# bowang-lab/BioReason

Hardware: AMD Instinct MI355X
Metric: GRPO samples/sec (NT-500M+Qwen3-1.7B, DNA 2x1024, prompt 2180, gen 256) (higher is better)
Workload: dtype bf16

## Files before the change

### bioreason_amd/csrc/bra_decattn.h

```cpp
#pragma once
#include "bra_device.h"
#include "bra_gridsync.h"

namespace bra {


constexpr float kNegA = -1.0e30f;
constexpr float kLog2eA = 1.4426950408889634f;

struct DecOneArgs {
    const bf16_t* qkv; long ldqkv;
    const bf16_t* qw; const bf16_t* kw;
    const float* cosT; const float* sinT;
    const int* pos;
    const float* rope_rows;
    const bf16_t* kp; long kp_sr, kp_sh, kp_ss;
    const bf16_t* vtp; long vt_sr, vt_sh, vt_sd;
    const uint8_t* pmask;
    bf16_t* kc;
    bf16_t* vct; long cp;
    float* part_o; float* part_ml;
    bf16_t* o; long ldo;
    int R, copies, Hq, Hkv, P, C, t, nslot, npc, ncc_grid;
    float eps, scale;
    const int* t_ptr;
    float inv_Hq, inv_npc, inv_Hkv, inv_ncc, inv_copies;
    int rsplit; float inv_rsplit;
};

__device__ __forceinline__ int da_div(int w, float inv) { return (int)(((float)w + 0.5f) * inv); }
#ifdef BRA_EMU
__device__ __forceinline__ unsigned da_mul24(int a, int b) { return ((unsigned)a & 0xffffffu) * ((unsigned)b & 0xffffffu); }
#else
__device__ __forceinline__ unsigned da_mul24(int a, int b) { return __umul24((unsigned)a, (unsigned)b); }
#endif

template <int HD>
__device__ __forceinline__ void nr_slice(float (&x)[8], const bf16_t* nw, const float* cosr, const float* sinr, int dl, float eps) {
    constexpr int LPK = HD / 8;
    float ss = 0.f;
#pragma unroll
    for (int i = 0; i < 8; ++i) ss += x[i] * x[i];
#pragma unroll
    for (int mk = LPK >> 1; mk >= 1; mk >>= 1) ss += wave_shfl_xor(ss, mk);
    const float rstd = rsqrtf(ss / (float)HD + eps);
    float w[8];
    unpack8(ld16(nw + dl * 8), w);
#pragma unroll
    for (int i = 0; i < 8; ++i) x[i] = round_bf(w[i] * round_bf(x[i] * rstd));
    const int hsl = (dl & (LPK / 2 - 1)) * 8;
    const bool upper = dl >= LPK / 2;
    const f32x4 c0 = *reinterpret_cast<const f32x4*>(cosr + hsl), c1 = *reinterpret_cast<const f32x4*>(cosr + hsl + 4);
    const f32x4 s0 = *reinterpret_cast<const f32x4*>(sinr + hsl), s1 = *reinterpret_cast<const f32x4*>(sinr + hsl + 4);
#pragma unroll
    for (int i = 0; i < 8; ++i) {
        const float other = wave_shfl_xor(x[i], LPK / 2);
        const float c = i < 4 ? c0[i & 3] : c1[i & 3], s = i < 4 ? s0[i & 3] : s1[i & 3];
        x[i] = round_bf(upper ? x[i] * c + other * s : x[i] * c - other * s);
    }
}

template <int HD>
__device__ __forceinline__ void item_kv_issue(const bf16_t* kbase, const int kss, const bf16_t* vbase, const int vsd, const int key0,
                                              const int nkeys, u32x4 (&kf)[4][HD / 32], u32x4 (&vf)[HD / 16][2]) {
    constexpr int DS = HD / 32, DB = HD / 16;
    const int lane = lane_id();
    const int fr = lane & 15, fq = lane >> 4;
#pragma unroll
    for (int kb = 0; kb < 4; ++kb) {
        int key = key0 + 32 * (kb >> 1) + 8 * (fr >> 2) + 4 * (kb & 1) + (fr & 3);
        key = key < nkeys ? key : nkeys - 1;
        const bf16_t* kr = kbase + (da_mul24(key, kss) + (unsigned)(fq * 8));
#pragma unroll
        for (int s = 0; s < DS; ++s) kf[kb][s] = ld16(kr + s * 32);
    }
    const unsigned vlane = da_mul24(fr, vsd) + (unsigned)(key0 + fq * 8);
#pragma unroll
    for (int db = 0; db < DB; ++db) {
        const bf16_t* vr = vbase + (long)db * 16 * vsd + vlane;
#pragma unroll
        for (int kk = 0; kk < 2; ++kk) vf[db][kk] = ld16(vr + kk * 32);
    }
}

template <int HD, int G, int XS = 0, int PRE = 0>
__device__ __forceinline__ void one_item(const DecOneArgs& a, const bf16_t* kbase, const int kss, const bf16_t* vbase, const int vsd,
                                         const int key0, const int nkeys, const uint8_t* mask, const int r, const int hkv,
                                         const int row_lo, const int row_hi, const int slot,
                                         u32x4 (&kf)[4][HD / 32], u32x4 (&vf)[HD / 16][2]) {
    constexpr int DS = HD / 32;
    constexpr int DB = HD / 16;
    const int lane = lane_id();
    const int fr = lane & 15, fq = lane >> 4;
    const int rows = a.copies * G;
    const int qrow = fr < rows ? fr : rows - 1;
    const int copy = (int)((unsigned)qrow / (unsigned)G), g = (int)((unsigned)qrow % (unsigned)G);
    const int b = r * a.copies + copy, hq = hkv * G + g;
    const unsigned qoff = da_mul24(b, (int)a.ldqkv) + (unsigned)(hq * HD);
    u32x4 qraw[DS], qwv[DS];
#pragma unroll
    for (int s = 0; s < DS; ++s) qraw[s] = xld16<XS>(a.qkv, (qoff + (unsigned)(s * 32 + fq * 8)) * 2u);
#pragma unroll
    for (int s = 0; s < DS; ++s) qwv[s] = ld16(a.qw + s * 32 + fq * 8);
    const float* cosr; const float* sinr;
    if (a.rope_rows) { cosr = a.rope_rows + (unsigned)(b * HD); sinr = cosr + HD / 2; }
    else { const int p = a.pos[b]; cosr = a.cosT + (long)p * (HD / 2); sinr = a.sinT + (long)p * (HD / 2); }
    f32x4 cs[DS / 2][4];
#pragma unroll
    for (int s = 0; s < DS / 2; ++s) {
        const int hb = s * 32 + fq * 8;
        cs[s][0] = *reinterpret_cast<const f32x4*>(cosr + hb); cs[s][1] = *reinterpret_cast<const f32x4*>(cosr + hb + 4);
        cs[s][2] = *reinterpret_cast<const f32x4*>(sinr + hb); cs[s][3] = *reinterpret_cast<const f32x4*>(sinr + hb + 4);
    }
    const bool nomask = mask == nullptr;
    uint8_t mb;
    {
        const int key = key0 + lane;
        const uint8_t* mp = nomask ? reinterpret_cast<const uint8_t*>(a.qw) : mask + (unsigned)(key < nkeys ? key : nkeys - 1);
        mb = *mp;
    }
    if constexpr (PRE == 0) item_kv_issue<HD>(kbase, kss, vbase, vsd, key0, nkeys, kf, vf);
    uint64_t vbits;
    {
        const int key = key0 + lane;
        vbits = wave_ballot((key < nkeys) & (nomask | (mb != 0)));
    }
    sched_fence();
    float qv[DS][8];
    float ss = 0.f;
#pragma unroll
    for (int s = 0; s < DS; ++s) {
        unpack8(qraw[s], qv[s]);
#pragma unroll
        for (int i = 0; i < 8; ++i) ss += qv[s][i] * qv[s][i];
    }
    ss += wave_shfl_xor(ss, 16);
    ss += wave_shfl_xor(ss, 32);
    const float rstd = rsqrtf(ss / (float)HD + a.eps);
#pragma unroll
    for (int s = 0; s < DS; ++s) {
        float w[8];
        unpack8(qwv[s], w);
#pragma unroll
        for (int i = 0; i < 8; ++i) qv[s][i] = round_bf(w[i] * round_bf(qv[s][i] * rstd));
    }
    const float sc = a.scale * kLog2eA;
    u32x4 qf[DS];
#pragma unroll
    for (int s = 0; s < DS; ++s) {
        const bool upper = s >= DS / 2;
        const int sp = s ^ (DS / 2), sh = s & (DS / 2 - 1);
        float o[8];
#pragma unroll
        for (int i = 0; i < 8; ++i) {
            const float cv = i < 4 ? cs[sh][0][i & 3] : cs[sh][1][i & 3], sv = i < 4 ? cs[sh][2][i & 3] : cs[sh][3][i & 3];
            const float rot = upper ? qv[s][i] * cv + qv[sp][i] * sv : qv[s][i] * cv - qv[sp][i] * sv;
            o[i] = round_bf(rot) * sc;
        }
        qf[s] = pack8(o);
    }
    f32x4 sreg[4];
    float m = kNegA;
#pragma unroll
    for (int kb = 0; kb < 4; ++kb) {
        f32x4 acc = {0.f, 0.f, 0.f, 0.f};
#pragma unroll
        for (int s = 0; s < DS; ++s) acc = mfma_16x16x32(kf[kb][s], qf[s], acc);
#pragma unroll
        for (int j = 0; j < 4; ++j) {
            const int rel_ = 32 * (kb >> 1) + 8 * fq + 4 * (kb & 1) + j;
            const bool ok = (vbits >> rel_) & 1ull;
            acc[j] = ok ? acc[j] : kNegA;
            m = fmaxf(m, acc[j]);
        }
        sreg[kb] = acc;
    }
    m = fmaxf(m, wave_shfl_xor(m, 16));
    m = fmaxf(m, wave_shfl_xor(m, 32));
    float l = 0.f;
#pragma unroll
    for (int kb = 0; kb < 4; ++kb)
#pragma unroll
        for (int j = 0; j < 4; ++j) {
            const float pe = sreg[kb][j] > 0.5f * kNegA ? fast_exp2(sreg[kb][j] - m) : 0.f;
            sreg[kb][j] = pe;
            l += pe;
        }
    l += wave_shfl_xor(l, 16);
    l += wave_shfl_xor(l, 32);
    const unsigned base = da_mul24((int)da_mul24(b, a.Hq) + hq, a.nslot) + (unsigned)slot;
    const bool live = fr < rows && fr >= row_lo && fr < row_hi;
#pragma unroll
    for (int db = 0; db < DB; ++db) {
        f32x4 acc = {0.f, 0.f, 0.f, 0.f};
#pragma unroll
        for (int kk = 0; kk < 2; ++kk) {
            u32x4 pf;
            pf.x = pack_bf2(sreg[2 * kk][0], sreg[2 * kk][1]);
            pf.y = pack_bf2(sreg[2 * kk][2], sreg[2 * kk][3]);
            pf.z = pack_bf2(sreg[2 * kk + 1][0], sreg[2 * kk + 1][1]);
            pf.w = pack_bf2(sreg[2 * kk + 1][2], sreg[2 * kk + 1][3]);
            acc = mfma_16x16x32(vf[db][kk], pf, acc);
        }
        if (live) xst16<XS>(a.part_o, (base * HD + (unsigned)(db * 16 + 4 * fq)) * 4u, __builtin_bit_cast(u32x4, acc));
    }
    if (live && fq == 0) {
        u32x2 mlv; mlv.x = __builtin_bit_cast(uint32_t, m); mlv.y = __builtin_bit_cast(uint32_t, l);
        xst8<XS>(a.part_ml, base * 8u, mlv);
    }
}

template <int HD, int G, int XS = 0>
__device__ __forceinline__ void one_newkey(const DecOneArgs& a, const int b, const int hq, const int t) {
    constexpr int LPK = HD / 8;
    const int lane = lane_id();
    const int grp = lane / LPK, dl = lane % LPK;
    const int hkv = hq / G;
    const int Nq = a.Hq * HD, Nkv = a.Hkv * HD;
    const int which = grp == 1 ? 1 : (grp == 2 ? 2 : 0);
    const unsigned src = da_mul24(b, (int)a.ldqkv) + (unsigned)(which == 0 ? hq * HD : (which == 1 ? Nq + hkv * HD : Nq + Nkv + hkv * HD));
    float x[8], y[8];
    unpack8(xld16<XS>(a.qkv, (src + (unsigned)(dl * 8)) * 2u), x);
    const float* cosr; const float* sinr;
    if (a.rope_rows) { cosr = a.rope_rows + (long)b * HD; sinr = cosr + HD / 2; }
    else { const int p = a.pos[b]; cosr = a.cosT + (long)p * (HD / 2); sinr = a.sinT + (long)p * (HD / 2); }
#pragma unroll
    for (int i = 0; i < 8; ++i) y[i] = x[i];
    nr_slice<HD>(y, which == 1 ? a.kw : a.qw, cosr, sinr, dl, a.eps);
    float d = 0.f;
#pragma unroll
    for (int i = 0; i < 8; ++i) d += y[i] * wave_shfl_xor(y[i], LPK);
#pragma unroll
    for (int mk = LPK >> 1; mk >= 1; mk >>= 1) d += wave_shfl_xor(d, mk);
    const float s_new = wave_shfl(d, 0) * a.scale * kLog2eA;
    if (hq % G == 0) {
        if (grp == 1) st16(a.kc + (((long)b * a.Hkv + hkv) * a.C + t) * HD + dl * 8, pack8(y));
        if (grp == 2) {
            bf16_t* vp = a.vct + (((long)b * a.Hkv + hkv) * HD + dl * 8) * a.cp + t;
#pragma unroll
            for (int i = 0; i < 8; ++i) vp[(long)i * a.cp] = f2bf(x[i]);
        }
    }
    const unsigned base = (unsigned)((b * a.Hq + hq) * a.nslot + a.npc + (t + 63) / 64);
    if (grp == 2) {
        const unsigned ob = (base * HD + (unsigned)(dl * 8)) * 4u;
        xst16<XS>(a.part_o, ob, __builtin_bit_cast(u32x4, f32x4{x[0], x[1], x[2], x[3]}));
        xst16<XS>(a.part_o, ob + 16u, __builtin_bit_cast(u32x4, f32x4{x[4], x[5], x[6], x[7]}));
    }
    if (lane == 0) {
        u32x2 mlv; mlv.x = __builtin_bit_cast(uint32_t, s_new); mlv.y = __builtin_bit_cast(uint32_t, 1.f);
        xst8<XS>(a.part_ml, base * 8u, mlv);
    }
}

struct DecItem {
    int kind;
    int b, hq;
    const bf16_t* kbase; int kss; const bf16_t* vbase; int vsd; int key0, nkeys; const uint8_t* mask;
    int r, hkv, row_lo, row_hi, slot;
};

template <int HD, int G>
__device__ __forceinline__ void dec_item_decode(const DecOneArgs& a, int w, const int t, DecItem& d) {
    const int nK = a.R * a.copies * a.Hq;
    const int nP = a.npc * a.Hkv * a.R;
    d.kind = 0;
    if (w >= nK && w < nK + nP) {
        w -= nK;
        const int q1 = da_div(w, a.inv_npc), c = w - q1 * a.npc;
        const int r = da_div(q1, a.inv_Hkv), hkv = q1 - r * a.Hkv;
        const int rp = a.rsplit > 1 ? da_div(r, a.inv_rsplit) : r;
        d.kind = 2;
        d.kbase = a.kp + rp * a.kp_sr + hkv * a.kp_sh; d.kss = (int)a.kp_ss;
        d.vbase = a.vtp + rp * a.vt_sr + hkv * a.vt_sh; d.vsd = (int)a.vt_sd;
        d.key0 = c * 64; d.nkeys = a.P; d.mask = a.pmask ? a.pmask + (long)rp * a.P : nullptr;
        d.r = r; d.hkv = hkv; d.row_lo = 0; d.row_hi = 16; d.slot = c;
        return;
    }
    if (w < nK) {
        d.kind = 1;
        d.b = da_div(w, a.inv_Hq);
        d.hq = w - d.b * a.Hq;
        return;
    }
    {
        const int v = w - nK - nP;
        const int q1 = da_div(v, a.inv_ncc), c = v - q1 * a.ncc_grid;
        const int q2 = da_div(q1, a.inv_copies), copy = q1 - q2 * a.copies;
        const int r = da_div(q2, a.inv_Hkv), hkv = q2 - r * a.Hkv;
        if (c * 64 >= t || r >= a.R) return;
        const int b = r * a.copies + copy;
        d.kind = 2;
        d.kbase = a.kc + ((long)b * a.Hkv + hkv) * a.C * HD; d.kss = HD;
        d.vbase = a.vct + ((long)b * a.Hkv + hkv) * HD * a.cp; d.vsd = (int)a.cp;
        d.key0 = c * 64; d.nkeys = t; d.mask = nullptr;
        d.r = r; d.hkv = hkv; d.row_lo = copy * G; d.row_hi = copy * G + G; d.slot = a.npc + c;
    }
}

template <int HD, int G, int XS, int PRE>
__device__ __forceinline__ void dec_item_run(const DecOneArgs& a, const DecItem& d, const int t, u32x4 (&kf)[4][HD / 32], u32x4 (&vf)[HD / 16][2]) {
    if (d.kind == 2)
        one_item<HD, G, XS, PRE>(a, d.kbase, d.kss, d.vbase, d.vsd, d.key0, d.nkeys, d.mask, d.r, d.hkv, d.row_lo, d.row_hi, d.slot, kf, vf);
    else if (d.kind == 1)
        one_newkey<HD, G, XS>(a, d.b, d.hq, t);
}

template <int HD, int G, int XS = 0>
__device__ __forceinline__ void dec_attn_item(const DecOneArgs& a, int w) {
    u32x4 kf[4][HD / 32], vf[HD / 16][2];
    const int nK = a.R * a.copies * a.Hq, nP = a.npc * a.Hkv * a.R;
    const int t = (w >= nK && w < nK + nP) ? 0 : (a.t_ptr ? a.t_ptr[0] : a.t);
    DecItem d;
    dec_item_decode<HD, G>(a, w, t, d);
    dec_item_run<HD, G, XS, 0>(a, d, t, kf, vf);
}

#ifdef BRA_EMU
__device__ __forceinline__ void da_pin(uint32_t&) {}
#else
__device__ __forceinline__ void da_pin(uint32_t& v) { asm volatile("" : "+v"(v)); }
#endif

__device__ __forceinline__ float da_ror_f(float v, int n) {
    const uint32_t u = __builtin_bit_cast(uint32_t, v);
    const uint32_t r = n == 8 ? row_ror_u32<8>(u) : (n == 4 ? row_ror_u32<4>(u) : (n == 2 ? row_ror_u32<2>(u) : row_ror_u32<1>(u)));
    return __builtin_bit_cast(float, r);
}
__device__ __forceinline__ float da_wave_max(float v) {
    v = fmaxf(v, da_ror_f(v, 8)); v = fmaxf(v, da_ror_f(v, 4)); v = fmaxf(v, da_ror_f(v, 2)); v = fmaxf(v, da_ror_f(v, 1));
    v = fmaxf(v, wave_shfl_xor(v, 16));
    return fmaxf(v, wave_shfl_xor(v, 32));
}
__device__ __forceinline__ float da_wave_sum(float v) {
    v += da_ror_f(v, 8); v += da_ror_f(v, 4); v += da_ror_f(v, 2); v += da_ror_f(v, 1);
    v += wave_shfl_xor(v, 16);
    return v + wave_shfl_xor(v, 32);
}

struct DaNoHook { __device__ __forceinline__ void operator()() const {} };

template <int HD, int XS = 0, class Hook = DaNoHook>
__device__ __forceinline__ void dec_attn_merge_one(const DecOneArgs& a, const int hq, const int b, const Hook& after_issue = Hook()) {
    constexpr int LR = HD / 4, PR = 64 / LR, PRE = 24;
    const int lane = lane_id();
    const int t = a.t_ptr ? a.t_ptr[0] : a.t;
    const int nsl = a.npc + (t + 63) / 64 + 1;
    const int p = lane / LR, d4 = lane % LR;
    const unsigned base = (unsigned)((b * a.Hq + hq) * a.nslot);
    u32x2 mlw[4];
#pragma unroll
    for (int q4 = 0; q4 < 4; ++q4) {
        const int c = lane + 64 * q4;
        mlw[q4] = xld8<XS>(a.part_ml, (base * 2u + (unsigned)((c < nsl ? c : nsl - 1) * 2)) * 4u);
    }
    u32x4 v0[PRE];
#pragma unroll
    for (int u = 0; u < PRE; ++u) {
        const int c = u * PR + p;
        v0[u] = xld16<XS>(a.part_o, (base * HD + (unsigned)((c < nsl ? c : nsl - 1) * HD + d4 * 4)) * 4u);
    }
    sched_fence();
    after_issue();
    float mc[4], lc[4];
#pragma unroll
    for (int q4 = 0; q4 < 4; ++q4) {
        uint32_t wm = mlw[q4].x, wl = mlw[q4].y;
        da_pin(wm); da_pin(wl);
        mc[q4] = __builtin_bit_cast(float, wm);
        lc[q4] = __builtin_bit_cast(float, wl);
    }
    float m = kNegA;
#pragma unroll
    for (int q4 = 0; q4 < 4; ++q4) {
        if (lane + 64 * q4 >= nsl) { mc[q4] = kNegA; lc[q4] = 0.f; }
        m = fmaxf(m, mc[q4]);
    }
    m = da_wave_max(m);
    float l = 0.f;
#pragma unroll
    for (int q4 = 0; q4 < 4; ++q4) { mc[q4] = fast_exp2(mc[q4] - m); l += lc[q4] * mc[q4]; }
    l = da_wave_sum(l);
    float acc[4] = {0.f, 0.f, 0.f, 0.f};
#pragma unroll
    for (int u = 0; u < PRE; ++u) {
        const int c = u * PR + p;
        const float wsel = (c >> 6) == 0 ? mc[0] : mc[1];
        float w = wave_shfl(wsel, c & 63);
        w = c < nsl ? w : 0.f;
        const f32x4 ov = __builtin_bit_cast(f32x4, v0[u]);
#pragma unroll
        for (int j = 0; j < 4; ++j) acc[j] += w * ov[j];
    }
    for (int c0 = PRE * PR; c0 < nsl; c0 += 8 * PR) {
        u32x4 v[8];
        float w[8];
#pragma unroll
        for (int u = 0; u < 8; ++u) {
            const int c = c0 + u * PR + p;
            const int cc = c < nsl ? c : nsl - 1;
            v[u] = xld16<XS>(a.part_o, ((base + (unsigned)cc) * HD + (unsigned)(d4 * 4)) * 4u);
            const float wsel = (cc >> 6) == 0 ? mc[0] : ((cc >> 6) == 1 ? mc[1] : ((cc >> 6) == 2 ? mc[2] : mc[3]));
            w[u] = wave_shfl(wsel, cc & 63);
            w[u] = c < nsl ? w[u] : 0.f;
        }
#pragma unroll
        for (int u = 0; u < 8; ++u) {
            const f32x4 ov = __builtin_bit_cast(f32x4, v[u]);
#pragma unroll
            for (int j = 0; j < 4; ++j) acc[j] += w[u] * ov[j];
        }
    }
#pragma unroll
    for (int mk = LR; mk < 64; mk <<= 1)
#pragma unroll
        for (int j = 0; j < 4; ++j) acc[j] += wave_shfl_xor(acc[j], mk);
    const float inv = l > 0.f ? 1.f / l : 0.f;
    if (p == 0) {
        u32x2 ov;
        ov.x = pack_bf2(acc[0] * inv, acc[1] * inv);
        ov.y = pack_bf2(acc[2] * inv, acc[3] * inv);
        xst8<XS>(a.o, (da_mul24(b, (int)a.ldo) + (unsigned)(hq * HD + d4 * 4)) * 2u, ov);
    }
}


}
```

### bioreason_amd/csrc/k_decattn.hip

```cpp
#include "bra_decattn.h"
#include "bra_api_internal.h"

namespace bra {

template <int HD, int G>
__global__ __launch_bounds__(64) void dec_attn_items_kernel(DecOneArgs a) {
    dec_attn_item<HD, G, 0>(a, (int)blockIdx.x);
}

template <int HD>
__global__ __launch_bounds__(64) void dec_attn_merge_kernel(float* m_part_ml, float* m_part_o, bf16_t* m_o, int m_ldo, int m_Hq, int m_nslot,
                                                            int m_npc, int m_t, const int* m_t_ptr, DecOneArgs a0) {
    DecOneArgs a = a0;
    a.part_ml = m_part_ml; a.part_o = m_part_o; a.o = m_o; a.ldo = m_ldo; a.Hq = m_Hq; a.nslot = m_nslot; a.npc = m_npc; a.t = m_t; a.t_ptr = m_t_ptr;
    dec_attn_merge_one<HD, 0>(a, (int)blockIdx.x, (int)blockIdx.y);
}

}

using namespace bra;

extern "C" int bra_dec_attn_one(const void* qkv, long ldqkv, const void* qw, const void* kw, const float* cosT, const float* sinT,
                                const int* pos, const float* rope_rows, const void* kp, long kp_sr, long kp_sh, long kp_ss,
                                const void* vtp, long vt_sr, long vt_sh, long vt_sd, const void* pmask, void* kc, void* vct, long cp,
                                float* part_o, float* part_ml, int nslot, void* o, long ldo, int R, int copies,
                                int Hq, int Hkv, int hd, int P, int C, int t, float eps, float scale, const int* t_dev, void* stream) {
    if (R <= 0 || copies <= 0 || Hq <= 0 || Hkv <= 0 || Hq % Hkv || P <= 0 || t < 0 || t >= C) return BRA_ERR_ARG;
    const int G = Hq / Hkv;
    int rsplit = 1;
    while (rsplit <= copies && (copies % rsplit || (copies / rsplit) * G > 16)) ++rsplit;
    if (rsplit > copies || G > 16) return BRA_ERR_UNSUPPORTED;
    const int R_phys = R;
    R *= rsplit; copies /= rsplit;
    (void)R_phys;
    if (!qkv || !qw || !kw || !cosT || !sinT || !pos || !kp || !vtp || !kc || !vct || !part_o || !part_ml || !o) return BRA_ERR_ARG;
    const int npc = (P + 63) / 64, ncc = (t + 63) / 64;
    if (vt_sd < (long)npc * 64 || vt_sd % 8 || kp_ss % 8 || cp < ((C + 63) / 64) * 64 || cp % 8 || ldqkv % 8 || ldo % 4) return BRA_ERR_ARG;
    if (nslot < npc + (C + 63) / 64 + 1 || nslot > 256) return BRA_ERR_ARG;
    DecOneArgs a = {(const bf16_t*)qkv, ldqkv, (const bf16_t*)qw, (const bf16_t*)kw, cosT, sinT, pos, rope_rows,
                    (const bf16_t*)kp, kp_sr, kp_sh, kp_ss, (const bf16_t*)vtp, vt_sr, vt_sh, vt_sd, (const uint8_t*)pmask,
                    (bf16_t*)kc, (bf16_t*)vct, cp, part_o, part_ml, (bf16_t*)o, ldo,
                    R, copies, Hq, Hkv, P, C, t, nslot, npc, ncc, eps, scale, t_dev,
                    1.f / (float)Hq, 1.f / (float)npc, 1.f / (float)Hkv, 1.f / (float)(ncc > 0 ? ncc : 1), 1.f / (float)copies,
                    rsplit, 1.f / (float)rsplit};
    bra_stream_t st = (bra_stream_t)stream;
    const int nitems = npc * Hkv * R + ncc * copies * Hkv * R + R * copies * Hq;
    const long lim = 1L << 30, f24 = 1L << 24;
    const long Bq = (long)R * copies;
    if (nitems >= (1 << 21) || kp_ss >= f24 || vt_sd >= f24 || cp >= f24 || ldqkv >= f24 || (long)(npc * 64) * kp_ss >= lim ||
        (long)hd * vt_sd >= lim || (long)hd * cp >= lim || Bq * ldqkv >= lim || Bq * Hq * nslot * hd >= lim || Bq * hd >= lim)
        return BRA_ERR_UNSUPPORTED;
#define BRA_DO(HD_, G_)                                                                                   \
    if (hd == HD_ && G == G_) {                                                                           \
        BRA_LAUNCH((dec_attn_items_kernel<HD_, G_>), dim3(nitems), dim3(64), 0, st, a);                   \
        BRA_LAUNCH((dec_attn_merge_kernel<HD_>), dim3(Hq, R * copies), dim3(64), 0, st, a.part_ml, a.part_o, a.o, (int)a.ldo, a.Hq,   \
                   a.nslot, a.npc, a.t, a.t_ptr, a);                                                      \
        return BRA_LAUNCH_STATUS();                                                                       \
    }
    BRA_DO(128, 1) BRA_DO(128, 2) BRA_DO(128, 4) BRA_DO(64, 1) BRA_DO(64, 2) BRA_DO(64, 4)
#undef BRA_DO
    return BRA_ERR_UNSUPPORTED;
}
```

### bioreason_amd/csrc/k_persist.hip

```cpp
#define BRA_LANE_OPAQUE 1
#include "bra_gridsync.h"
#include "bra_decattn.h"
#include "bra_decgemm.h"
#include "bra_api_internal.h"

namespace bra {

#ifndef BRA_EMU
template <int NT>
__global__ __launch_bounds__(NT) void gridbar_probe_kernel(GridSync* gs, unsigned* buf , unsigned* errs,
                                                           const u32x4* wts, unsigned long wts_chunks, int iters, int mode_in,
                                                           int wchunks, unsigned timeout_ticks) {
    int mode = mode_in;
    __shared__ unsigned flag;
    const int nwg = (int)gridDim.x, wg = (int)blockIdx.x, tid = (int)threadIdx.x;
    unsigned epoch = 0, bad = 0, sink = 0;
    const __amdgpu_buffer_rsrc_t rs = xs_rsrc(buf);
    const unsigned nwords = (unsigned)nwg * 32u;
    for (int it = 0; it < iters; ++it) {
        unsigned* slot = buf + (size_t)(it & 1) * nwords;
        u32x4 w[8];
        const bool spoll = mode >= 4;
        if (mode == 5) mode = 3;
        if (mode == 4) mode = 1;
// ... 178 lines not shown
                                        const u32x2& resv, const f32x4 (&sq)[8], float (&red)[2][8][64][4], float (&rs_lds)[8],
                                        const int wave, const int lane) {
    const int fr = lane & 15;
    if (wave < NW) {
        f32x4 acc = {0.f, 0.f, 0.f, 0.f};
#pragma unroll
        for (int u = 0; u < NL; ++u) acc = mfma_16x16x32(w.v[u], x.v[u], acc);
        if (NORM == 2 && it == 0 && wave == 0) {
            const float rs = dg2_fold_rstd(sq, g.nss_in >> 3, g.inv_K, g.eps);
            if ((lane & 7) == 0) rs_lds[lane >> 3] = rs;
        }
#pragma unroll
        for (int r = 0; r < 4; ++r) red[it & 1][wave][lane][r] = acc[r];
    }
    raw_barrier();
    if (wave == it % NW) {
        float v[4];
        dg2_reduce<NW>(red[it & 1], lane, v);
        if (NORM == 2) {
            const int mrow = MODE ? (fr & 7) : fr;
            const float rsf = rs_lds[mrow < g.M ? mrow : g.M - 1];
#pragma unroll
            for (int r = 0; r < 4; ++r) v[r] *= rsf;
        }
        dg2_epilogue<MODE, ACT, 0, 1, 1>(g, v, tile, lane, true, resv);
    }
}

template <int H, int NQ, int NKV, int F, int HD, int G, int PF>
__global__ __launch_bounds__(512) void decode_persist_kernel(PersistArgs a) {
    constexpr int NQKV = NQ + 2 * NKV;
    constexpr int NWG = NQKV / 16;
    constexpr int NL_QKV = H / 256;
    constexpr int NW_O = (NQ / 64 >= 64) ? 8 : 4, NL_O = NQ / 64 / NW_O;
    constexpr int NL_D = F / 64 / 8;
    constexpr int NT_GU = 2 * F / 16 / NWG;
    constexpr int GU_A = 3;
    static_assert(H % 256 == 0 && (NL_QKV == 4 || NL_QKV == 8 || NL_QKV == 12), "qkv / gate-up: one register round of 8 waves");
    static_assert(H / 8 == NWG && (2 * F / 16) % NWG == 0 && NT_GU == 3, "tiles per workgroup: 1 qkv, 1 o, 3 gate/up, 1 down");
    static_assert(NQ % (64 * NW_O) == 0 && (NL_O == 4 || NL_O == 8 || NL_O == 12) && F % 512 == 0 && (NL_D == 4 || NL_D == 8 || NL_D == 12), "o / down");
    __shared__ float red[2][8][64][4];
    __shared__ float rs_lds[8];
    __shared__ unsigned bar_flag;
#define BRA_PIDS()                                                                                             \
    int wave, wg;                                                                                              \
    { int tw_ = (int)threadIdx.x >> 6; asm volatile("" : "+v"(tw_)); wave = __builtin_amdgcn_readfirstlane(tw_);   \
      wg = (int)blockIdx.x; asm volatile("" : "+s"(wg)); }
    unsigned epoch = 0;
    int phases = 0;
    const int M = a.M;
    DecOneArgs at = a.att;
    const int t = at.t_ptr ? at.t_ptr[0] : at.t;
    at.t = t; at.t_ptr = nullptr;
    {
        const int ncc = (t + 63) / 64;
        at.ncc_grid = ncc; at.inv_ncc = 1.f / (float)(ncc > 0 ? ncc : 1);
    }
    const int nitems = at.R * at.copies * at.Hq + at.npc * at.Hkv * at.R + at.ncc_grid * at.copies * at.Hkv * at.R;
    const u32x2 zero2 = {0u, 0u};
    f32x4 sq0[8];
#pragma unroll
    for (int i = 0; i < 8; ++i) sq0[i] = f32x4{0.f, 0.f, 0.f, 0.f};
    Frag<NL_QKV> wq;
#define BRA_PSTAMP(k_)                                                                        \
    do {                                                                                      \
        if (a.stamps && blockIdx.x == 0 && threadIdx.x == 0) a.stamps[phases * 4 + (k_)] = __builtin_amdgcn_s_memrealtime(); \
    } while (0)
#define BRA_PRUN() (PF > 0 || (phases >= a.ph_lo && phases < a.ph_hi))
#define BRA_PBAR()                                                                            \
    do {                                                                                      \
        const bool both_ = PF > 0 || (phases >= a.ph_lo && phases + 1 < a.ph_hi);             \
        ++phases;                                                                             \
        if (phases >= a.ph_hi) return;                                                        \
        if (both_ && !grid_barrier(a.sync, epoch, NWG, a.timeout_ticks, &bar_flag)) return;   \
    } while (0)
    const PLayer* Ls = a.layers;
    if (PF) { BRA_PIDS(); pw_issue<8, NL_QKV>(wq, Ls[0].Wqkv, wg, wave, lane_id()); sched_fence(); }
    for (int l = 0; l < a.L; ++l) {
        const PLayer Lr = Ls[l];
        Frag<NL_QKV> wg0, wg1;
        Frag<NL_O> wo;
        Frag<NL_D> wd;
        at.qw = Lr.qn; at.kw = Lr.kn; at.kp = Lr.kp; at.vtp = Lr.vtp; at.kc = Lr.kc; at.vct = Lr.vct;
        {
            u32x4 kf[4][HD / 32], vf[HD / 16][2];
            DecItem it0;
            it0.kind = 0;
            if (BRA_PRUN()) {
            BRA_PIDS();
            DecGemm2Args g = {a.x, H, a.ssx, a.nss, nullptr, a.eps, Lr.Wqkv, H, nullptr, 0, (void*)at.qkv, NQKV, nullptr, 0, M, NQKV, H, 3, nullptr, nullptr, 1.f / (float)H};
            if (PF >= 2) {
                const int iw = wg + NWG * wave;
                if (iw < nitems) dec_item_decode<HD, G>(at, iw, t, it0);
                if (it0.kind == 2) item_kv_issue<HD>(it0.kbase, it0.kss, it0.vbase, it0.vsd, it0.key0, it0.nkeys, kf, vf);
                sched_fence();
            }
            BRA_PSTAMP(0);
            if (!PF) pw_issue<8, NL_QKV>(wq, Lr.Wqkv, wg, wave, lane_id());
            Frag<NL_QKV> xf;
            px_load<0, 8, NL_QKV>(xf, a.x, H, M, wave, lane_id());
            f32x4 sq[8];
            ps_load(sq, a.ssx, a.nss, M, wave, lane_id());
            pg_tile<0, 2, 0, 8, NL_QKV>(wq, xf, g, wg, 0, zero2, sq, red, rs_lds, wave, lane_id());
            BRA_PSTAMP(2);
            if (wave == 0) gs_drain();
            BRA_PSTAMP(3);
            }
            BRA_PBAR();
          if (BRA_PRUN()) {
            BRA_PIDS();
            BRA_PSTAMP(0);
            if (PF >= 2) {
                if (wg + NWG * wave < nitems) dec_item_run<HD, G, 1, 1>(at, it0, t, kf, vf);
                for (int i = wg + NWG * (wave + 8); i < nitems; i += NWG * 8) {
                    DecItem d;
                    dec_item_decode<HD, G>(at, i, t, d);
                    dec_item_run<HD, G, 1, 0>(at, d, t, kf, vf);
                }
            } else {
                for (int i = wg + NWG * wave; i < nitems; i += NWG * 8) {
                    DecItem d;
                    dec_item_decode<HD, G>(at, i, t, d);
                    dec_item_run<HD, G, 1, 0>(at, d, t, kf, vf);
                }
            }
            BRA_PSTAMP(2);
            gs_drain();
            BRA_PSTAMP(3);
          }
            BRA_PBAR();
        }
        if (BRA_PRUN()) {
        BRA_PIDS();
        BRA_PSTAMP(0);
        auto look_ahead = [&]() {
            if (PF) {
                pw_issue<NW_O, NL_O>(wo, Lr.Wo, wg, wave, lane_id());
                pw_issue<8, NL_QKV, 0, GU_A>(wg0, Lr.Wgu, wg, wave, lane_id());
                sched_fence();
            }
        };
        {
            const int i = wg + NWG * wave;
            if (i < M * at.Hq) {
                const int b = da_div(i, at.inv_Hq);
                dec_attn_merge_one<HD, 1>(at, i - b * at.Hq, b);
            }
        }
        BRA_PSTAMP(2);
        gs_drain();
        if (PF) {
            bare_barrier();
            sched_fence();
            look_ahead();
        }
        BRA_PSTAMP(3);
        }
        BRA_PBAR();
        {
            if (BRA_PRUN()) {
            BRA_PIDS();
            BRA_PSTAMP(0);
            DecGemm2Args g = {at.o, NQ, nullptr, 0, nullptr, 0.f, Lr.Wo, NQ, a.x, H, (void*)a.h, H, a.ssh, a.nss, M, H, NQ, 1, nullptr, nullptr, 1.f / (float)NQ};
            if (!PF) pw_issue<NW_O, NL_O>(wo, Lr.Wo, wg, wave, lane_id());
            Frag<NL_O> xf;
            px_load<1, NW_O, NL_O>(xf, at.o, NQ, M, wave, lane_id());
            const u32x2 resv = pr_load<1>(a.x, H, M, H, wg, lane_id());
            pg_tile<1, 0, 0, NW_O, NL_O>(wo, xf, g, wg, 0, resv, sq0, red, rs_lds, wave, lane_id());
            BRA_PSTAMP(2);
            if (wave == 0) gs_drain();
            if (PF) {
                bare_barrier();
                sched_fence();
                pw_issue<8, NL_D, 0, NL_D / 2>(wd, Lr.Wd, wg, wave, lane_id());
                sched_fence();
            }
// ... 202 lines not shown
```

### include/bioreason_hip_debug.h

```cpp
#ifndef BIOREASON_HIP_DEBUG_H
#define BIOREASON_HIP_DEBUG_H
#include "bioreason_hip.h"
#ifdef __cplusplus
extern "C" {
#endif

int bra_gemm_set_variant(int v);
int bra_gemm_set_ring_fill(int pct);
int bra_gemm_set_row_split(int on);
int bra_gemm_set_epi_lds(int on);
int bra_sample_set_one_launch(int on);
int bra_gemm_set_glds_rows(int rows);
int bra_attn_set_block_order(int legacy);
int bra_attn_set_fwd4(int on);
int bra_attn_set_bwd4(int mask);
int bra_attn_set_probe(void* buf);


int bra_dec_gemm2_probe(const void* x, long ldx, const float* ss_in, int nss_in, const void* norm_w, float eps, const void* W,
                        long ldw, const void* res, long ldres, void* out, long ldo, float* ss_out, int nss_out, int M, int N,
                        int K, int act, int out_f32, int packed, void* probe, void* stream);
int bra_debug_set_probe(void* p);

int bra_gridsync_bytes(void);
int bra_persist_layer_desc_size(void);
int bra_persist_set_stamps(void* p);
int bra_qwen_layers_persist(const void* layers_dev, int L, int R, int copies, int H, int Hq, int Hkv, int hd, int F, int P,
                            long vt_pitch, int C, long cp, float eps, float scale, const float* cosT, const float* sinT,
                            const int* pos, const float* rope_rows, const void* pmask, int t, const int* t_dev, void* x,
                            void* qkv, void* o, void* h, void* act, float* ss_ws, int nss, float* part_o, float* part_ml,
                            int nslot, void* sync, int prefetch, int stop_after, int timeout_us, void* stream);
int bra_qwen_decode_step_persist(const void* layers_host, const void* layers_dev, int L, int R, int copies, int H, int Hq, int Hkv,
                                 int hd, int F, int P, long vt_pitch, int C, long cp, int V, float eps, float scale, const void* E,
                                 const void* norm_w, const float* cosT, const float* sinT, const int* tok, const int* pos,
                                 const void* pmask, int t, const int* t_dev, int embed_done, void* x, void* qkv, void* o, void* h,
                                 void* act, float* ss_ws, int nss, float* part_o, float* part_ml, int nslot, float* logits,
                                 void* sync, int prefetch, int stop_after, int timeout_us, void* stream);
int bra_chain_probe(void* done, void* buf, void* errs, const void* wts, long wts_bytes, int nwg, int n, int chained, int wchunks,
                    int timeout_us, void* stream_a, void* stream_b);
int bra_gridbar_probe(void* sync, void* buf, void* errs, const void* wts, long wts_bytes, int nwg, int iters, int mode,
                      int wchunks, int timeout_us, void* stream);

#ifdef __cplusplus
}
#endif
#endif
```

Before: 19.43.

## Group two 64-key chunks per decode attention work item and adapt merge

Each split-K decode attention item now processes two 64-key chunks (for both prompt and generated cache) instead of one. This halves the number of partial slots and items, reducing per-item overhead (q norm/rope recompute, partial writes) and the merge work. The merge kernel gains a fast path when the slot count fits in one wave. The trade-off is more registers per item and fewer parallel items, which could hurt occupancy or load balance.

```diff
diff --git a/bioreason_amd/csrc/bra_decattn.h b/bioreason_amd/csrc/bra_decattn.h
--- a/bioreason_amd/csrc/bra_decattn.h
+++ b/bioreason_amd/csrc/bra_decattn.h
@@ -26,7 +26,15 @@
     const int* t_ptr;
     float inv_Hq, inv_npc, inv_Hkv, inv_ncc, inv_copies;
     int rsplit; float inv_rsplit;
+    int npg, lgc; float inv_npg;
 };
+
+constexpr int kChP = 2, kChC = 2;
+__host__ __device__ inline int da_ncg(int t, int lgc) { return (((t + 63) >> 6) + (1 << lgc) - 1) >> lgc; }
+__host__ __device__ inline void da_set_groups(DecOneArgs& a, int chp, int lgc, int t_grid) {
+    a.npg = (a.npc + chp - 1) / chp; a.inv_npg = 1.f / (float)a.npg; a.lgc = lgc;
+    a.ncc_grid = da_ncg(t_grid, lgc); a.inv_ncc = 1.f / (float)(a.ncc_grid > 0 ? a.ncc_grid : 1);
+}
 
 __device__ __forceinline__ int da_div(int w, float inv) { return (int)(((float)w + 0.5f) * inv); }
 #ifdef BRA_EMU
@@ -74,7 +82,9 @@
 #pragma unroll
         for (int s = 0; s < DS; ++s) kf[kb][s] = ld16(kr + s * 32);
     }
-    const unsigned vlane = da_mul24(fr, vsd) + (unsigned)(key0 + fq * 8);
+    const int lastc = ((nkeys - 1) >> 6) << 6;
+    const int key0v = key0 < lastc ? key0 : lastc;
+    const unsigned vlane = da_mul24(fr, vsd) + (unsigned)(key0v + fq * 8);
 #pragma unroll
     for (int db = 0; db < DB; ++db) {
         const bf16_t* vr = vbase + (long)db * 16 * vsd + vlane;
@@ -83,11 +93,12 @@
     }
 }
 
-template <int HD, int G, int XS = 0, int PRE = 0>
+template <int HD, int G, int XS, int PRE, int CH, int CHM>
 __device__ __forceinline__ void one_item(const DecOneArgs& a, const bf16_t* kbase, const int kss, const bf16_t* vbase, const int vsd,
                                          const int key0, const int nkeys, const uint8_t* mask, const int r, const int hkv,
                                          const int row_lo, const int row_hi, const int slot,
-                                         u32x4 (&kf)[4][HD / 32], u32x4 (&vf)[HD / 16][2]) {
+                                         u32x4 (&kf)[CHM][4][HD / 32], u32x4 (&vf)[CHM][HD / 16][2]) {
+    static_assert(CH >= 1 && CH <= CHM, "chunk group");
     constexpr int DS = HD / 32;
     constexpr int DB = HD / 16;
     const int lane = lane_id();
@@ -113,17 +124,20 @@
         cs[s][2] = *reinterpret_cast<const f32x4*>(sinr + hb); cs[s][3] = *reinterpret_cast<const f32x4*>(sinr + hb + 4);
     }
     const bool nomask = mask == nullptr;
-    uint8_t mb;
-    {
-        const int key = key0 + lane;
+    uint8_t mb[CH];
+#pragma unroll
+    for (int j = 0; j < CH; ++j) {
+        const int key = key0 + 64 * j + lane;
         const uint8_t* mp = nomask ? reinterpret_cast<const uint8_t*>(a.qw) : mask + (unsigned)(key < nkeys ? key : nkeys - 1);
-        mb = *mp;
-    }
-    if constexpr (PRE == 0) item_kv_issue<HD>(kbase, kss, vbase, vsd, key0, nkeys, kf, vf);
-    uint64_t vbits;
-    {
-        const int key = key0 + lane;
-        vbits = wave_ballot((key < nkeys) & (nomask | (mb != 0)));
+        mb[j] = *mp;
+    }
+#pragma unroll
+    for (int j = PRE ? 1 : 0; j < CH; ++j) item_kv_issue<HD>(kbase, kss, vbase, vsd, key0 + 64 * j, nkeys, kf[j], vf[j]);
+    uint64_t vbits[CH];
+#pragma unroll
+    for (int j = 0; j < CH; ++j) {
+        const int key = key0 + 64 * j + lane;
+        vbits[j] = wave_ballot((key < nkeys) & (nomask | (mb[j] != 0)));
     }
     sched_fence();
     float qv[DS][8];
@@ -159,49 +173,58 @@
         }
         qf[s] = pack8(o);
     }
-    f32x4 sreg[4];
+    f32x4 sreg[CH][4];
     float m = kNegA;
 #pragma unroll
-    for (int kb = 0; kb < 4; ++kb) {
-        f32x4 acc = {0.f, 0.f, 0.f, 0.f};
-#pragma unroll
-        for (int s = 0; s < DS; ++s) acc = mfma_16x16x32(kf[kb][s], qf[s], acc);
-#pragma unroll
-        for (int j = 0; j < 4; ++j) {
-            const int rel_ = 32 * (kb >> 1) + 8 * fq + 4 * (kb & 1) + j;
-            const bool ok = (vbits >> rel_) & 1ull;
-            acc[j] = ok ? acc[j] : kNegA;
-            m = fmaxf(m, acc[j]);
-        }
-        sreg[kb] = acc;
-    }
+    for (int c = 0; c < CH; ++c)
+#pragma unroll
+        for (int kb = 0; kb < 4; ++kb) {
+            f32x4 acc = {0.f, 0.f, 0.f, 0.f};
+#pragma unroll
+            for (int s = 0; s < DS; ++s) acc = mfma_16x16x32(kf[c][kb][s], qf[s], acc);
+#pragma unroll
+            for (int j = 0; j < 4; ++j) {
+                const int rel_ = 32 * (kb >> 1) + 8 * fq + 4 * (kb & 1) + j;
+                const bool ok = (vbits[c] >> rel_) & 1ull;
+                acc[j] = ok ? acc[j] : kNegA;
+                m = fmaxf(m, acc[j]);
+            }
+            sreg[c][kb] = acc;
+        }
     m = fmaxf(m, wave_shfl_xor(m, 16));
     m = fmaxf(m, wave_shfl_xor(m, 32));
     float l = 0.f;
 #pragma unroll
-    for (int kb = 0; kb < 4; ++kb)
-#pragma unroll
-        for (int j = 0; j < 4; ++j) {
-            const float pe = sreg[kb][j] > 0.5f * kNegA ? fast_exp2(sreg[kb][j] - m) : 0.f;
-            sreg[kb][j] = pe;
-            l += pe;
-        }
+    for (int c = 0; c < CH; ++c)
+#pragma unroll
+        for (int kb = 0; kb < 4; ++kb)
+#pragma unroll
+            for (int j = 0; j < 4; ++j) {
+                const float pe = sreg[c][kb][j] > 0.5f * kNegA ? fast_exp2(sreg[c][kb][j] - m) : 0.f;
+                sreg[c][kb][j] = pe;
+                l += pe;
+            }
     l += wave_shfl_xor(l, 16);
     l += wave_shfl_xor(l, 32);
     const unsigned base = da_mul24((int)da_mul24(b, a.Hq) + hq, a.nslot) + (unsigned)slot;
     const bool live = fr < rows && fr >= row_lo && fr < row_hi;
+    u32x4 pf[CH][2];
+#pragma unroll
+    for (int c = 0; c < CH; ++c)
+#pragma unroll
+        for (int kk = 0; kk < 2; ++kk) {
+            pf[c][kk].x = pack_bf2(sreg[c][2 * kk][0], sreg[c][2 * kk][1]);
+            pf[c][kk].y = pack_bf2(sreg[c][2 * kk][2], sreg[c][2 * kk][3]);
+            pf[c][kk].z = pack_bf2(sreg[c][2 * kk + 1][0], sreg[c][2 * kk + 1][1]);
+            pf[c][kk].w = pack_bf2(sreg[c][2 * kk + 1][2], sreg[c][2 * kk + 1][3]);
+        }
 #pragma unroll
     for (int db = 0; db < DB; ++db) {
         f32x4 acc = {0.f, 0.f, 0.f, 0.f};
 #pragma unroll
-        for (int kk = 0; kk < 2; ++kk) {
-            u32x4 pf;
-            pf.x = pack_bf2(sreg[2 * kk][0], sreg[2 * kk][1]);
-            pf.y = pack_bf2(sreg[2 * kk][2], sreg[2 * kk][3]);
-            pf.z = pack_bf2(sreg[2 * kk + 1][0], sreg[2 * kk + 1][1]);
-            pf.w = pack_bf2(sreg[2 * kk + 1][2], sreg[2 * kk + 1][3]);
-            acc = mfma_16x16x32(vf[db][kk], pf, acc);
-        }
+        for (int c = 0; c < CH; ++c)
+#pragma unroll
+            for (int kk = 0; kk < 2; ++kk) acc = mfma_16x16x32(vf[c][db][kk], pf[c][kk], acc);
         if (live) xst16<XS>(a.part_o, (base * HD + (unsigned)(db * 16 + 4 * fq)) * 4u, __builtin_bit_cast(u32x4, acc));
     }
     if (live && fq == 0) {
@@ -241,7 +264,7 @@
             for (int i = 0; i < 8; ++i) vp[(long)i * a.cp] = f2bf(x[i]);
         }
     }
-    const unsigned base = (unsigned)((b * a.Hq + hq) * a.nslot + a.npc + (t + 63) / 64);
+    const unsigned base = (unsigned)((b * a.Hq + hq) * a.nslot + a.npg + da_ncg(t, a.lgc));
     if (grp == 2) {
         const unsigned ob = (base * HD + (unsigned)(dl * 8)) * 4u;
         xst16<XS>(a.part_o, ob, __builtin_bit_cast(u32x4, f32x4{x[0], x[1], x[2], x[3]}));
@@ -260,27 +283,22 @@
     int r, hkv, row_lo, row_hi, slot;
 };
 
-template <int HD, int G>
+template <int HD, int G, int CHP, int CHC>
 __device__ __forceinline__ void dec_item_decode(const DecOneArgs& a, int w, const int t, DecItem& d) {
     const int nK = a.R * a.copies * a.Hq;
-    const int nP = a.npc * a.Hkv * a.R;
-    d.kind = 0;
+    const int nP = a.npg * a.Hkv * a.R;
     if (w >= nK && w < nK + nP) {
         w -= nK;
-        const int q1 = da_div(w, a.inv_npc), c = w - q1 * a.npc;
+        const int q1 = da_div(w, a.inv_npg), c = w - q1 * a.npg;
         const int r = da_div(q1, a.inv_Hkv), hkv = q1 - r * a.Hkv;
         const int rp = a.rsplit > 1 ? da_div(r, a.inv_rsplit) : r;
-        d.kind = 2;
-        d.kbase = a.kp + rp * a.kp_sr + hkv * a.kp_sh; d.kss = (int)a.kp_ss;
-        d.vbase = a.vtp + rp * a.vt_sr + hkv * a.vt_sh; d.vsd = (int)a.vt_sd;
-        d.key0 = c * 64; d.nkeys = a.P; d.mask = a.pmask ? a.pmask + (long)rp * a.P : nullptr;
-        d.r = r; d.hkv = hkv; d.row_lo = 0; d.row_hi = 16; d.slot = c;
+        d = DecItem{2, 0, 0, a.kp + rp * a.kp_sr + hkv * a.kp_sh, (int)a.kp_ss, a.vtp + rp * a.vt_sr + hkv * a.vt_sh, (int)a.vt_sd,
+                    c * (64 * CHP), a.P, a.pmask ? a.pmask + (long)rp * a.P : nullptr, r, hkv, 0, 16, c};
         return;
     }
     if (w < nK) {
-        d.kind = 1;
-        d.b = da_div(w, a.inv_Hq);
-        d.hq = w - d.b * a.Hq;
+        const int b = da_div(w, a.inv_Hq);
+        d = DecItem{1, b, w - b * a.Hq, nullptr, 0, nullptr, 0, 0, 0, nullptr, 0, 0, 0, 0, 0};
         return;
     }
     {
@@ -288,32 +306,37 @@
         const int q1 = da_div(v, a.inv_ncc), c = v - q1 * a.ncc_grid;
         const int q2 = da_div(q1, a.inv_copies), copy = q1 - q2 * a.copies;
         const int r = da_div(q2, a.inv_Hkv), hkv = q2 - r * a.Hkv;
-        if (c * 64 >= t || r >= a.R) return;
+        if (c * (64 * CHC) >= t || r >= a.R) {
+            d = DecItem{0, 0, 0, nullptr, 0, nullptr, 0, 0, 0, nullptr, 0, 0, 0, 0, 0};
+            return;
+        }
         const int b = r * a.copies + copy;
-        d.kind = 2;
-        d.kbase = a.kc + ((long)b * a.Hkv + hkv) * a.C * HD; d.kss = HD;
-        d.vbase = a.vct + ((long)b * a.Hkv + hkv) * HD * a.cp; d.vsd = (int)a.cp;
-        d.key0 = c * 64; d.nkeys = t; d.mask = nullptr;
-        d.r = r; d.hkv = hkv; d.row_lo = copy * G; d.row_hi = copy * G + G; d.slot = a.npc + c;
-    }
-}
-
-template <int HD, int G, int XS, int PRE>
-__device__ __forceinline__ void dec_item_run(const DecOneArgs& a, const DecItem& d, const int t, u32x4 (&kf)[4][HD / 32], u32x4 (&vf)[HD / 16][2]) {
-    if (d.kind == 2)
-        one_item<HD, G, XS, PRE>(a, d.kbase, d.kss, d.vbase, d.vsd, d.key0, d.nkeys, d.mask, d.r, d.hkv, d.row_lo, d.row_hi, d.slot, kf, vf);
+        d = DecItem{3, 0, 0, a.kc + ((long)b * a.Hkv + hkv) * a.C * HD, HD, a.vct + ((long)b * a.Hkv + hkv) * HD * a.cp, (int)a.cp,
+                    c * (64 * CHC), t, nullptr, r, hkv, copy * G, copy * G + G, a.npg + c};
+    }
+}
+
+template <int HD, int G, int XS, int PRE, int CHP, int CHC>
+__device__ __forceinline__ void dec_item_run(const DecOneArgs& a, const DecItem& d, const int t,
+                                             u32x4 (&kf)[(CHP > CHC ? CHP : CHC)][4][HD / 32], u32x4 (&vf)[(CHP > CHC ? CHP : CHC)][HD / 16][2]) {
+    constexpr int CHM = CHP > CHC ? CHP : CHC;
+    if (CHP == CHC ? d.kind >= 2 : d.kind == 2)
+        one_item<HD, G, XS, PRE, CHP, CHM>(a, d.kbase, d.kss, d.vbase, d.vsd, d.key0, d.nkeys, d.mask, d.r, d.hkv, d.row_lo, d.row_hi, d.slot, kf, vf);
+    else if (d.kind == 3)
+        one_item<HD, G, XS, PRE, CHC, CHM>(a, d.kbase, d.kss, d.vbase, d.vsd, d.key0, d.nkeys, d.mask, d.r, d.hkv, d.row_lo, d.row_hi, d.slot, kf, vf);
     else if (d.kind == 1)
         one_newkey<HD, G, XS>(a, d.b, d.hq, t);
 }
 
-template <int HD, int G, int XS = 0>
+template <int HD, int G, int XS, int CHP, int CHC>
 __device__ __forceinline__ void dec_attn_item(const DecOneArgs& a, int w) {
-    u32x4 kf[4][HD / 32], vf[HD / 16][2];
-    const int nK = a.R * a.copies * a.Hq, nP = a.npc * a.Hkv * a.R;
+    constexpr int CHM = CHP > CHC ? CHP : CHC;
+    u32x4 kf[CHM][4][HD / 32], vf[CHM][HD / 16][2];
+    const int nK = a.R * a.copies * a.Hq, nP = a.npg * a.Hkv * a.R;
     const int t = (w >= nK && w < nK + nP) ? 0 : (a.t_ptr ? a.t_ptr[0] : a.t);
     DecItem d;
-    dec_item_decode<HD, G>(a, w, t, d);
-    dec_item_run<HD, G, XS, 0>(a, d, t, kf, vf);
+    dec_item_decode<HD, G, CHP, CHC>(a, w, t, d);
+    dec_item_run<HD, G, XS, 0, CHP, CHC>(a, d, t, kf, vf);
 }
 
 #ifdef BRA_EMU
@@ -340,17 +363,16 @@
 
 struct DaNoHook { __device__ __forceinline__ void operator()() const {} };
 
-template <int HD, int XS = 0, class Hook = DaNoHook>
-__device__ __forceinline__ void dec_attn_merge_one(const DecOneArgs& a, const int hq, const int b, const Hook& after_issue = Hook()) {
-    constexpr int LR = HD / 4, PR = 64 / LR, PRE = 24;
+template <int HD, int XS, int NML, int PRE, class Hook>
+__device__ __forceinline__ void dec_attn_merge_body(const DecOneArgs& a, const int hq, const int b, const int nsl, const Hook& after_issue) {
+    constexpr int LR = HD / 4, PR = 64 / LR;
+    static_assert(PRE * PR <= 64 * NML, "weights of the up-front rows");
     const int lane = lane_id();
-    const int t = a.t_ptr ? a.t_ptr[0] : a.t;
-    const int nsl = a.npc + (t + 63) / 64 + 1;
     const int p = lane / LR, d4 = lane % LR;
     const unsigned base = (unsigned)((b * a.Hq + hq) * a.nslot);
-    u32x2 mlw[4];
-#pragma unroll
-    for (int q4 = 0; q4 < 4; ++q4) {
+    u32x2 mlw[NML];
+#pragma unroll
+    for (int q4 = 0; q4 < NML; ++q4) {
         const int c = lane + 64 * q4;
         mlw[q4] = xld8<XS>(a.part_ml, (base * 2u + (unsigned)((c < nsl ? c : nsl - 1) * 2)) * 4u);
     }
@@ -362,9 +384,9 @@
     }
     sched_fence();
     after_issue();
-    float mc[4], lc[4];
-#pragma unroll
-    for (int q4 = 0; q4 < 4; ++q4) {
+    float mc[NML], lc[NML];
+#pragma unroll
+    for (int q4 = 0; q4 < NML; ++q4) {
         uint32_t wm = mlw[q4].x, wl = mlw[q4].y;
         da_pin(wm); da_pin(wl);
         mc[q4] = __builtin_bit_cast(float, wm);
@@ -372,21 +394,20 @@
     }
     float m = kNegA;
 #pragma unroll
-    for (int q4 = 0; q4 < 4; ++q4) {
+    for (int q4 = 0; q4 < NML; ++q4) {
         if (lane + 64 * q4 >= nsl) { mc[q4] = kNegA; lc[q4] = 0.f; }
         m = fmaxf(m, mc[q4]);
     }
     m = da_wave_max(m);
     float l = 0.f;
 #pragma unroll
-    for (int q4 = 0; q4 < 4; ++q4) { mc[q4] = fast_exp2(mc[q4] - m); l += lc[q4] * mc[q4]; }
+    for (int q4 = 0; q4 < NML; ++q4) { mc[q4] = fast_exp2(mc[q4] - m); l += lc[q4] * mc[q4]; }
     l = da_wave_sum(l);
     float acc[4] = {0.f, 0.f, 0.f, 0.f};
 #pragma unroll
     for (int u = 0; u < PRE; ++u) {
         const int c = u * PR + p;
-        const float wsel = (c >> 6) == 0 ? mc[0] : mc[1];
-        float w = wave_shfl(wsel, c & 63);
+        float w = wave_shfl(mc[(u * PR) >> 6], c & 63);
         w = c < nsl ? w : 0.f;
         const f32x4 ov = __builtin_bit_cast(f32x4, v0[u]);
 #pragma unroll
@@ -400,7 +421,9 @@
             const int c = c0 + u * PR + p;
             const int cc = c < nsl ? c : nsl - 1;
             v[u] = xld16<XS>(a.part_o, ((base + (unsigned)cc) * HD + (unsigned)(d4 * 4)) * 4u);
-            const float wsel = (cc >> 6) == 0 ? mc[0] : ((cc >> 6) == 1 ? mc[1] : ((cc >> 6) == 2 ? mc[2] : mc[3]));
+            float wsel = mc[0];
+#pragma unroll
+            for (int q4 = 1; q4 < NML; ++q4) wsel = (cc >> 6) == q4 ? mc[q4] : wsel;
             w[u] = wave_shfl(wsel, cc & 63);
             w[u] = c < nsl ? w[u] : 0.f;
         }
@@ -424,5 +447,14 @@
     }
 }
 
-
-}
+template <int HD, int XS = 0, class Hook = DaNoHook>
+__device__ __forceinline__ void dec_attn_merge_one(const DecOneArgs& a, const int hq, const int b, const Hook& after_issue = Hook()) {
+    constexpr int PR = 256 / HD;
+    const int t = a.t_ptr ? a.t_ptr[0] : a.t;
+    const int nsl = a.npg + da_ncg(t, a.lgc) + 1;
+    if (nsl <= 64) dec_attn_merge_body<HD, XS, 1, 22 / PR, Hook>(a, hq, b, nsl, after_issue);
+    else dec_attn_merge_body<HD, XS, 4, 24, Hook>(a, hq, b, nsl, after_issue);
+}
+
+
+}
diff --git a/bioreason_amd/csrc/k_decattn.hip b/bioreason_amd/csrc/k_decattn.hip
--- a/bioreason_amd/csrc/k_decattn.hip
+++ b/bioreason_amd/csrc/k_decattn.hip
@@ -1,24 +1,40 @@
 #include "bra_decattn.h"
 #include "bra_api_internal.h"
+#include <atomic>
 
 namespace bra {
 
-template <int HD, int G>
+template <int HD, int G, int CHP, int CHC>
 __global__ __launch_bounds__(64) void dec_attn_items_kernel(DecOneArgs a) {
-    dec_attn_item<HD, G, 0>(a, (int)blockIdx.x);
+    dec_attn_item<HD, G, 0, CHP, CHC>(a, (int)blockIdx.x);
 }
 
 template <int HD>
 __global__ __launch_bounds__(64) void dec_attn_merge_kernel(float* m_part_ml, float* m_part_o, bf16_t* m_o, int m_ldo, int m_Hq, int m_nslot,
-                                                            int m_npc, int m_t, const int* m_t_ptr, DecOneArgs a0) {
+                                                            int m_npg, int m_t, int m_lgc, const int* m_t_ptr, DecOneArgs a0) {
     DecOneArgs a = a0;
-    a.part_ml = m_part_ml; a.part_o = m_part_o; a.o = m_o; a.ldo = m_ldo; a.Hq = m_Hq; a.nslot = m_nslot; a.npc = m_npc; a.t = m_t; a.t_ptr = m_t_ptr;
+    a.part_ml = m_part_ml; a.part_o = m_part_o; a.o = m_o; a.ldo = m_ldo; a.Hq = m_Hq; a.nslot = m_nslot; a.npg = m_npg; a.t = m_t; a.lgc = m_lgc;
+    a.t_ptr = m_t_ptr;
     dec_attn_merge_one<HD, 0>(a, (int)blockIdx.x, (int)blockIdx.y);
 }
 
 }
 
 using namespace bra;
+
+#ifdef BRA_DEBUG
+#ifdef BRA_EMU
+static int g_dec_attn_groups = kChP | (kChC << 8);
+#else
+static std::atomic<int> g_dec_attn_groups{kChP | (kChC << 8)};
+#endif
+extern "C" int bra_dec_attn_set_groups(int chp, int chc) {
+    if (chp <= 0 && chc <= 0) { g_dec_attn_groups = kChP | (kChC << 8); return BRA_OK; }
+    if ((chp != 1 && chp != 2) || (chc != 1 && chc != 2)) return BRA_ERR_ARG;
+    g_dec_attn_groups = chp | (chc << 8);
+    return BRA_OK;
+}
+#endif
 
 extern "C" int bra_dec_attn_one(const void* qkv, long ldqkv, const void* qw, const void* kw, const float* cosT, const float* sinT,
                                 const int* pos, const float* rope_rows, const void* kp, long kp_sr, long kp_sh, long kp_ss,
@@ -34,30 +50,43 @@
     R *= rsplit; copies /= rsplit;
     (void)R_phys;
     if (!qkv || !qw || !kw || !cosT || !sinT || !pos || !kp || !vtp || !kc || !vct || !part_o || !part_ml || !o) return BRA_ERR_ARG;
-    const int npc = (P + 63) / 64, ncc = (t + 63) / 64;
+    const int npc = (P + 63) / 64;
     if (vt_sd < (long)npc * 64 || vt_sd % 8 || kp_ss % 8 || cp < ((C + 63) / 64) * 64 || cp % 8 || ldqkv % 8 || ldo % 4) return BRA_ERR_ARG;
     if (nslot < npc + (C + 63) / 64 + 1 || nslot > 256) return BRA_ERR_ARG;
     DecOneArgs a = {(const bf16_t*)qkv, ldqkv, (const bf16_t*)qw, (const bf16_t*)kw, cosT, sinT, pos, rope_rows,
                     (const bf16_t*)kp, kp_sr, kp_sh, kp_ss, (const bf16_t*)vtp, vt_sr, vt_sh, vt_sd, (const uint8_t*)pmask,
                     (bf16_t*)kc, (bf16_t*)vct, cp, part_o, part_ml, (bf16_t*)o, ldo,
-                    R, copies, Hq, Hkv, P, C, t, nslot, npc, ncc, eps, scale, t_dev,
-                    1.f / (float)Hq, 1.f / (float)npc, 1.f / (float)Hkv, 1.f / (float)(ncc > 0 ? ncc : 1), 1.f / (float)copies,
-                    rsplit, 1.f / (float)rsplit};
+                    R, copies, Hq, Hkv, P, C, t, nslot, npc, 0, eps, scale, t_dev,
+                    1.f / (float)Hq, 1.f / (float)npc, 1.f / (float)Hkv, 1.f, 1.f / (float)copies,
+                    rsplit, 1.f / (float)rsplit, 0, 0, 1.f};
+#ifdef BRA_DEBUG
+    const int groups = g_dec_attn_groups;
+    const int chp = groups & 255, chc = groups >> 8;
+#else
+    constexpr int chp = kChP, chc = kChC;
+#endif
+    da_set_groups(a, chp, chc == 2 ? 1 : 0, t);
     bra_stream_t st = (bra_stream_t)stream;
-    const int nitems = npc * Hkv * R + ncc * copies * Hkv * R + R * copies * Hq;
+    const int nitems = a.npg * Hkv * R + a.ncc_grid * copies * Hkv * R + R * copies * Hq;
     const long lim = 1L << 30, f24 = 1L << 24;
     const long Bq = (long)R * copies;
     if (nitems >= (1 << 21) || kp_ss >= f24 || vt_sd >= f24 || cp >= f24 || ldqkv >= f24 || (long)(npc * 64) * kp_ss >= lim ||
         (long)hd * vt_sd >= lim || (long)hd * cp >= lim || Bq * ldqkv >= lim || Bq * Hq * nslot * hd >= lim || Bq * hd >= lim)
         return BRA_ERR_UNSUPPORTED;
-#define BRA_DO(HD_, G_)                                                                                   \
-    if (hd == HD_ && G == G_) {                                                                           \
-        BRA_LAUNCH((dec_attn_items_kernel<HD_, G_>), dim3(nitems), dim3(64), 0, st, a);                   \
+#define BRA_DO_CH(HD_, G_, CHP_, CHC_)                                                                    \
+    if (hd == HD_ && G == G_ && chp == CHP_ && chc == CHC_) {                                             \
+        BRA_LAUNCH((dec_attn_items_kernel<HD_, G_, CHP_, CHC_>), dim3(nitems), dim3(64), 0, st, a);       \
         BRA_LAUNCH((dec_attn_merge_kernel<HD_>), dim3(Hq, R * copies), dim3(64), 0, st, a.part_ml, a.part_o, a.o, (int)a.ldo, a.Hq,   \
-                   a.nslot, a.npc, a.t, a.t_ptr, a);                                                      \
+                   a.nslot, a.npg, a.t, a.lgc, a.t_ptr, a);                                               \
         return BRA_LAUNCH_STATUS();                                                                       \
     }
+#ifdef BRA_DEBUG
+#define BRA_DO(HD_, G_) BRA_DO_CH(HD_, G_, 1, 1) BRA_DO_CH(HD_, G_, 2, 1) BRA_DO_CH(HD_, G_, 1, 2) BRA_DO_CH(HD_, G_, 2, 2)
+#else
+#define BRA_DO(HD_, G_) BRA_DO_CH(HD_, G_, kChP, kChC)
+#endif
     BRA_DO(128, 1) BRA_DO(128, 2) BRA_DO(128, 4) BRA_DO(64, 1) BRA_DO(64, 2) BRA_DO(64, 4)
 #undef BRA_DO
+#undef BRA_DO_CH
     return BRA_ERR_UNSUPPORTED;
 }
diff --git a/bioreason_amd/csrc/k_persist.hip b/bioreason_amd/csrc/k_persist.hip
--- a/bioreason_amd/csrc/k_persist.hip
+++ b/bioreason_amd/csrc/k_persist.hip
@@ -254,11 +254,8 @@
     DecOneArgs at = a.att;
     const int t = at.t_ptr ? at.t_ptr[0] : at.t;
     at.t = t; at.t_ptr = nullptr;
-    {
-        const int ncc = (t + 63) / 64;
-        at.ncc_grid = ncc; at.inv_ncc = 1.f / (float)(ncc > 0 ? ncc : 1);
-    }
-    const int nitems = at.R * at.copies * at.Hq + at.npc * at.Hkv * at.R + at.ncc_grid * at.copies * at.Hkv * at.R;
+    da_set_groups(at, kChP, kChC == 2 ? 1 : 0, t);
+    const int nitems = at.R * at.copies * at.Hq + at.npg * at.Hkv * at.R + at.ncc_grid * at.copies * at.Hkv * at.R;
     const u32x2 zero2 = {0u, 0u};
     f32x4 sq0[8];
 #pragma unroll
@@ -285,7 +282,8 @@
         Frag<NL_D> wd;
         at.qw = Lr.qn; at.kw = Lr.kn; at.kp = Lr.kp; at.vtp = Lr.vtp; at.kc = Lr.kc; at.vct = Lr.vct;
         {
-            u32x4 kf[4][HD / 32], vf[HD / 16][2];
+            constexpr int CHM = kChP > kChC ? kChP : kChC;
+            u32x4 kf[CHM][4][HD / 32], vf[CHM][HD / 16][2];
             DecItem it0;
             it0.kind = 0;
             if (BRA_PRUN()) {
@@ -293,8 +291,8 @@
             DecGemm2Args g = {a.x, H, a.ssx, a.nss, nullptr, a.eps, Lr.Wqkv, H, nullptr, 0, (void*)at.qkv, NQKV, nullptr, 0, M, NQKV, H, 3, nullptr, nullptr, 1.f / (float)H};
             if (PF >= 2) {
                 const int iw = wg + NWG * wave;
-                if (iw < nitems) dec_item_decode<HD, G>(at, iw, t, it0);
-                if (it0.kind == 2) item_kv_issue<HD>(it0.kbase, it0.kss, it0.vbase, it0.vsd, it0.key0, it0.nkeys, kf, vf);
+                if (iw < nitems) dec_item_decode<HD, G, kChP, kChC>(at, iw, t, it0);
+                if (it0.kind >= 2) item_kv_issue<HD>(it0.kbase, it0.kss, it0.vbase, it0.vsd, it0.key0, it0.nkeys, kf[0], vf[0]);
                 sched_fence();
             }
             BRA_PSTAMP(0);
@@ -313,17 +311,17 @@
             BRA_PIDS();
             BRA_PSTAMP(0);
             if (PF >= 2) {
-                if (wg + NWG * wave < nitems) dec_item_run<HD, G, 1, 1>(at, it0, t, kf, vf);
+                if (wg + NWG * wave < nitems) dec_item_run<HD, G, 1, 1, kChP, kChC>(at, it0, t, kf, vf);
                 for (int i = wg + NWG * (wave + 8); i < nitems; i += NWG * 8) {
                     DecItem d;
-                    dec_item_decode<HD, G>(at, i, t, d);
-                    dec_item_run<HD, G, 1, 0>(at, d, t, kf, vf);
+                    dec_item_decode<HD, G, kChP, kChC>(at, i, t, d);
+                    dec_item_run<HD, G, 1, 0, kChP, kChC>(at, d, t, kf, vf);
                 }
             } else {
                 for (int i = wg + NWG * wave; i < nitems; i += NWG * 8) {
                     DecItem d;
-                    dec_item_decode<HD, G>(at, i, t, d);
-                    dec_item_run<HD, G, 1, 0>(at, d, t, kf, vf);
+                    dec_item_decode<HD, G, kChP, kChC>(at, i, t, d);
+                    dec_item_run<HD, G, 1, 0, kChP, kChC>(at, d, t, kf, vf);
                 }
             }
             BRA_PSTAMP(2);
diff --git a/include/bioreason_hip_debug.h b/include/bioreason_hip_debug.h
--- a/include/bioreason_hip_debug.h
+++ b/include/bioreason_hip_debug.h
@@ -21,6 +21,7 @@
                         long ldw, const void* res, long ldres, void* out, long ldo, float* ss_out, int nss_out, int M, int N,
                         int K, int act, int out_f32, int packed, void* probe, void* stream);
 int bra_debug_set_probe(void* p);
+int bra_dec_attn_set_groups(int chp, int chc);
 
 int bra_gridsync_bytes(void);
 int bra_persist_layer_desc_size(void);
```

New measurement: 19.36. About the same (-0.3%).
